# rcelha/rio-rs

Hardware: NVIDIA H100
Metric: placements/sec (higher is better)
Workload: dtype u32

## Files before the change

### rio_rs_b200/csrc/k_trie.cu

```cuda
#include "kernels.cuh"
#include "spec.cuh"
#include "bounded_tail.cuh"

#include <cstdlib>

namespace rio {

namespace {

constexpr int kTrieThreads = 256;
constexpr uint32_t kMaxLevels = 16;

__constant__ uint32_t c_lvl_s0[kMaxLevels];
__constant__ uint32_t c_lvl_m2[kMaxLevels];
__constant__ uint32_t c_lvl_h2[kMaxLevels];

__device__ __forceinline__ uint32_t smem_u32(const void *p) { return (uint32_t)__cvta_generic_to_shared(p); }

__device__ __forceinline__ void stage_blob_tma(void *smem_dst, const void *gsrc, uint32_t bytes, unsigned long long *bar) {
    if (threadIdx.x == 0) {
        asm volatile("mbarrier.init.shared::cta.b64 [%0], 1;" ::"r"(smem_u32(bar)) : "memory");
        asm volatile("fence.mbarrier_init.release.cluster;" ::: "memory");
    }
    __syncthreads();
    if (threadIdx.x == 0) {
        asm volatile("mbarrier.arrive.expect_tx.shared::cta.b64 _, [%0], %1;" ::"r"(smem_u32(bar)), "r"(bytes) : "memory");
        for (uint32_t off = 0; off < bytes; off += 32768u) {
            const uint32_t len = min(32768u, bytes - off);
            asm volatile("cp.async.bulk.shared::cluster.global.mbarrier::complete_tx::bytes [%0], [%1], %2, [%3];"
                         ::"r"(smem_u32(reinterpret_cast<unsigned char *>(smem_dst) + off)),
                           "l"(reinterpret_cast<const unsigned char *>(gsrc) + off), "r"(len), "r"(smem_u32(bar))
                         : "memory");
        }
    }
    uint32_t done = 0;
    while (!done) {
        asm volatile("{\n\t.reg .pred p;\n\tmbarrier.try_wait.parity.shared::cta.b64 p, [%1], %2;\n\tselp.u32 %0, 1, 0, p;\n\t}"
                     : "=r"(done) : "r"(smem_u32(bar)), "r"(0u) : "memory");
    }
}

__device__ __forceinline__ uint32_t walk_step(uint32_t off, uint32_t sel) {
    uint32_t r;
    asm("mad.lo.u32 %0, %1, 2, %2;" : "=r"(r) : "r"(off), "r"(sel));
    return r;
}

template <int BITS>
__device__ __forceinline__ uint32_t trie_leaf_index(ObjHash o, const uint32_t *__restrict__ tab32, uint32_t bits_rt) {
    uint32_t i = 1;
    if (BITS > 0) {
#pragma unroll
        for (int l = 0; l < BITS; l++) {
            const uint32_t u = contest_u(o, c_lvl_s0[l], c_lvl_m2[l], c_lvl_h2[l]);
            i = 2 * i + (u > tab32[i] ? 1u : 0u);
        }
    } else {
        for (uint32_t l = 0; l < bits_rt; l++) {
            const uint32_t u = contest_u(o, c_lvl_s0[l], c_lvl_m2[l], c_lvl_h2[l]);
            i = 2 * i + (u > tab32[i] ? 1u : 0u);
        }
    }
    return i;
}

__device__ __forceinline__ uint32_t trie_resolve_leaf(ObjHash o, uint32_t leaf, const unsigned char *__restrict__ blob) {
    if ((int32_t)leaf > -2) return leaf;
    uint32_t w = leaf;
    for (;;) {
        const unsigned char *p = blob + (w & 0x7FFFFFFFu);
        const uint4 r = *reinterpret_cast<const uint4 *>(p);
        const uint2 nn = *reinterpret_cast<const uint2 *>(p + 16);
        if (contest_u(o, r.x, r.y, r.z) <= r.w) return nn.x;
        if ((int32_t)nn.y >= 0) return nn.y;
        w = nn.y;
    }
}

struct TrieSmem {
    const uint32_t *tab32;
    const unsigned char *blob;
    uint32_t *hist;
};

template <bool SMEM>
__device__ __forceinline__ TrieSmem trie_stage(const TrieDev &t, uint32_t hist_bins) {
    extern __shared__ __align__(128) unsigned char smem_trie[];
    constexpr bool in_smem = SMEM;
    TrieSmem s;
    uint32_t off = 0;
    if (in_smem) {
        s.tab32 = reinterpret_cast<const uint32_t *>(smem_trie);
        s.blob = smem_trie;
        off = t.blob_bytes;
    } else {
        const unsigned char *g = reinterpret_cast<const unsigned char *>(t.blob);
        s.tab32 = reinterpret_cast<const uint32_t *>(g);
        s.blob = g;
    }
    s.hist = reinterpret_cast<uint32_t *>(smem_trie + off);
    for (uint32_t j = threadIdx.x; j < hist_bins; j += blockDim.x) s.hist[j] = 0;
    unsigned long long *bar = reinterpret_cast<unsigned long long *>(smem_trie + off + ((hist_bins * 4u + 15u) & ~15u));
    if (in_smem) stage_blob_tma(smem_trie, t.blob, t.blob_bytes, bar);
    else __syncthreads();
    return s;
}

template <int BITS, int OPT, int MODE, bool SMEM, int MINB = (SMEM ? 5 : 3)>
__global__ void __launch_bounds__(kTrieThreads, MINB)
k_assign_trie(const uint64_t *__restrict__ keys, uint64_t n, TrieDev t, uint32_t *__restrict__ out_idx, uint32_t *__restrict__ counters,
              uint32_t hist_bins, unsigned long long *__restrict__ moved, const __grid_constant__ BoundedTail tail) {
    static_assert(OPT % 2 == 0, "two objects per 128-bit load");
    constexpr bool in_smem = SMEM;
    constexpr int SEG = OPT / 2;
    const uint64_t tile_objs = (uint64_t)kTrieThreads * OPT;
    const uint64_t n_tiles = (n + tile_objs - 1) / tile_objs;
    unsigned long long n_moved = 0;
    ulonglong2 kk[SEG];
    auto load_tile = [&](uint64_t tile) {
        const uint64_t f0 = tile * tile_objs + 2 * threadIdx.x;
        if ((tile + 1) * tile_objs <= n) {
            const ulonglong2 *src = reinterpret_cast<const ulonglong2 *>(keys + f0);
#pragma unroll
            for (int g = 0; g < SEG; g++) kk[g] = __ldg(src + g * kTrieThreads);
            return;
        }
#pragma unroll
        for (int g = 0; g < SEG; g++) {
            const uint64_t f = f0 + (uint64_t)g * (2 * kTrieThreads);
            kk[g] = make_ulonglong2(0, 0);
            if (f + 1 < n) kk[g] = __ldg(reinterpret_cast<const ulonglong2 *>(keys + f));
            else if (f < n) kk[g].x = __ldg(keys + f);
        }
    };
    const TrieSmem s = trie_stage<SMEM>(t, hist_bins);
    asm volatile("griddepcontrol.launch_dependents;" ::: "memory");
    asm volatile("griddepcontrol.wait;" ::: "memory");
    if (blockIdx.x < n_tiles) load_tile(blockIdx.x);
    for (uint64_t tile = blockIdx.x; tile < n_tiles; tile += gridDim.x) {
        const uint64_t base = tile * tile_objs;
        const bool full_tile = base + tile_objs <= n;
        ObjHash o[OPT];
#pragma unroll
        for (int g = 0; g < SEG; g++) {
            o[2 * g] = obj_hash(kk[g].x);
            o[2 * g + 1] = obj_hash(kk[g].y);
        }
        if (tile + gridDim.x < n_tiles) load_tile(tile + gridDim.x);
        uint32_t leaf[OPT];
        if (in_smem) {
            const unsigned char *tb = reinterpret_cast<const unsigned char *>(s.tab32);
            uint32_t off[OPT];
#pragma unroll
            for (int k = 0; k < OPT; k++) off[k] = 4;
            if (BITS > 0) {
                constexpr int TOP = BITS >= 3 ? 3 : 0;
                if (TOP) {
#pragma unroll
                    for (int k = 0; k < OPT; k++) {
                        const bool c0 = contest_u(o[k], c_lvl_s0[0], c_lvl_m2[0], c_lvl_h2[0]) > t.top[1];
                        const bool c1 = contest_u(o[k], c_lvl_s0[1], c_lvl_m2[1], c_lvl_h2[1]) > (c0 ? t.top[3] : t.top[2]);
                        const uint32_t t2 = c0 ? (c1 ? t.top[7] : t.top[6]) : (c1 ? t.top[5] : t.top[4]);
                        const bool c2 = contest_u(o[k], c_lvl_s0[2], c_lvl_m2[2], c_lvl_h2[2]) > t2;
                        off[k] = 32u + (c0 ? 16u : 0u) + (c1 ? 8u : 0u) + (c2 ? 4u : 0u);
                    }
                }
#pragma unroll
                for (int l = TOP; l < BITS; l++) {
#pragma unroll
                    for (int k = 0; k < OPT; k++) {
                        const uint32_t u = contest_u(o[k], c_lvl_s0[l], c_lvl_m2[l], c_lvl_h2[l]);
                        const uint32_t thr = *reinterpret_cast<const uint32_t *>(tb + off[k]);
                        off[k] = walk_step(off[k], u > thr ? 4u : 0u);
                    }
                }
            } else {
                for (uint32_t l = 0; l < t.bits; l++) {
#pragma unroll
                    for (int k = 0; k < OPT; k++) {
                        const uint32_t u = contest_u(o[k], c_lvl_s0[l], c_lvl_m2[l], c_lvl_h2[l]);
                        const uint32_t thr = *reinterpret_cast<const uint32_t *>(tb + off[k]);
                        off[k] = walk_step(off[k], u > thr ? 4u : 0u);
                    }
                }
            }
#pragma unroll
            for (int k = 0; k < OPT; k++) leaf[k] = *reinterpret_cast<const uint32_t *>(tb + off[k]);
        } else {
#pragma unroll
            for (int k = 0; k < OPT; k++) leaf[k] = __ldg(s.tab32 + trie_leaf_index<0>(o[k], s.tab32, t.bits));
        }
        uint32_t nid[OPT];
#pragma unroll
        for (int k = 0; k < OPT; k++) nid[k] = trie_resolve_leaf(o[k], leaf[k], s.blob);
        if (MODE == 0 && full_tile) {
            uint2 *dst = reinterpret_cast<uint2 *>(out_idx + base + 2 * threadIdx.x);
#pragma unroll
            for (int g = 0; g < SEG; g++) dst[g * kTrieThreads] = make_uint2(nid[2 * g], nid[2 * g + 1]);
            if (counters && nid[0] != kNone) {
                if (hist_bins) {
#pragma unroll
                    for (int k = 0; k < OPT; k++) atomicAdd(&s.hist[nid[k]], 1u);
                } else {
#pragma unroll
                    for (int k = 0; k < OPT; k++) atomicAdd(&counters[nid[k]], 1u);
                }
            }
            continue;
        }
#pragma unroll
        for (int g = 0; g < SEG; g++) {
            const uint64_t first = base + (uint64_t)g * (2 * kTrieThreads) + 2 * threadIdx.x;
            if (first >= n) continue;
            const bool two = first + 1 < n;
            if (MODE == 1) {
                uint2 old = make_uint2(kNone, kNone);
                if (two) old = *reinterpret_cast<const uint2 *>(out_idx + first);
                else old.x = out_idx[first];
                const bool c0 = old.x != nid[2 * g], c1 = two && old.y != nid[2 * g + 1];
                if (c0 | c1) {
                    if (two) *reinterpret_cast<uint2 *>(out_idx + first) = make_uint2(nid[2 * g], nid[2 * g + 1]);
                    else out_idx[first] = nid[2 * g];
                }
                n_moved += (unsigned)c0 + (unsigned)c1;
            } else {
                if (two) *reinterpret_cast<uint2 *>(out_idx + first) = make_uint2(nid[2 * g], nid[2 * g + 1]);
                else out_idx[first] = nid[2 * g];
            }
            if (counters) {
                if (hist_bins) {
                    if (nid[2 * g] != kNone) atomicAdd(&s.hist[nid[2 * g]], 1u);
                    if (two && nid[2 * g + 1] != kNone) atomicAdd(&s.hist[nid[2 * g + 1]], 1u);
                } else {
                    if (nid[2 * g] != kNone) atomicAdd(&counters[nid[2 * g]], 1u);
                    if (two && nid[2 * g + 1] != kNone) atomicAdd(&counters[nid[2 * g + 1]], 1u);
                }
            }
        }
    }
    if (MODE == 1) {
#pragma unroll
        for (int sh = 16; sh > 0; sh >>= 1) n_moved += __shfl_xor_sync(0xFFFFFFFFu, n_moved, sh);
        if ((threadIdx.x & 31) == 0 && n_moved) atomicAdd(moved, n_moved);
    }
    if (hist_bins && counters) {
        __syncthreads();
        for (uint32_t j = threadIdx.x; j < hist_bins; j += blockDim.x) { const uint32_t v = s.hist[j]; if (v) atomicAdd(&counters[j], v); }
    }
    if (MODE == 0 && tail.enabled) {
        __shared__ uint32_t s_last;
        __threadfence();
        __syncthreads();
        if (threadIdx.x == 0) s_last = atomicAdd(tail.ticket, 1u) == gridDim.x - 1;
        __syncthreads();
        if (s_last) {
            if (threadIdx.x == 0) *tail.ticket = 0;
            __threadfence();
            exchange_and_check_block(tail, counters);
        }
    }
}

template <bool SMEM>
__global__ void __launch_bounds__(kTrieThreads, 4)
k_assign_trie_sel(const uint64_t *__restrict__ keys, const uint32_t *__restrict__ sel, uint64_t n_sel, TrieDev t, uint32_t *__restrict__ out_idx,
                  uint32_t *__restrict__ counters, uint32_t hist_bins) {
    const TrieSmem s = trie_stage<SMEM>(t, hist_bins);
    for (uint64_t q = (uint64_t)blockIdx.x * blockDim.x + threadIdx.x; q < n_sel; q += (uint64_t)gridDim.x * blockDim.x) {
        const uint32_t oi = __ldg(sel + q);
        const ObjHash o = obj_hash(__ldg(keys + oi));
        const uint32_t i = trie_leaf_index<0>(o, s.tab32, t.bits);
        const uint32_t nid = trie_resolve_leaf(o, s.tab32[i], s.blob);
        out_idx[oi] = nid;
        if (counters && nid != kNone) { if (hist_bins) atomicAdd(&s.hist[nid], 1u); else atomicAdd(&counters[nid], 1u); }
    }
    if (hist_bins && counters) {
        __syncthreads();
        for (uint32_t j = threadIdx.x; j < hist_bins; j += blockDim.x) { const uint32_t v = s.hist[j]; if (v) atomicAdd(&counters[j], v); }
    }
}

template <bool SMEM>
__global__ void __launch_bounds__(kTrieThreads, 4)
k_dir_reassign_trie(DirDev dir, TrieDev t, unsigned long long *__restrict__ moved) {
    const TrieSmem s = trie_stage<SMEM>(t, 0);
    const uint4 *slots = reinterpret_cast<const uint4 *>(dir.slots);
    const uint64_t cap = dir.mask + 1;
    unsigned long long n_moved = 0;
    for (uint64_t i = (uint64_t)blockIdx.x * blockDim.x + threadIdx.x; i < cap; i += (uint64_t)gridDim.x * blockDim.x) {
        const uint4 v = slots[i];
        const unsigned long long key = ((unsigned long long)v.y << 32) | v.x;
        if (key == kEmptyKey || v.z == kNone) continue;
        const ObjHash o = obj_hash(key);
        const uint32_t li = trie_leaf_index<0>(o, s.tab32, t.bits);
        const uint32_t nid = trie_resolve_leaf(o, s.tab32[li], s.blob);
        if (nid != v.z) { reinterpret_cast<uint32_t *>(&dir.slots[i].val)[0] = nid; n_moved++; }
    }
#pragma unroll
    for (int sh = 16; sh > 0; sh >>= 1) n_moved += __shfl_xor_sync(0xFFFFFFFFu, n_moved, sh);
    if ((threadIdx.x & 31) == 0 && n_moved) atomicAdd(moved, n_moved);
}

constexpr uint32_t kTrieSmemBudget = 200u * 1024u;

struct TrieLaunchShape { uint32_t hist_bins; uint32_t in_smem; size_t smem; int ctas_per_sm; };
TrieLaunchShape trie_shape(const TrieDev &t, bool want_hist, uint32_t n_total, int want_ctas) {
    TrieLaunchShape sh{};
    sh.hist_bins = (want_hist && n_total <= 8192) ? n_total : 0;
    const size_t tail = ((size_t)sh.hist_bins * 4 + 15) / 16 * 16 + 16;
    sh.in_smem = (t.blob_bytes + tail <= kTrieSmemBudget) ? 1u : 0u;
    sh.smem = (sh.in_smem ? t.blob_bytes : 0) + tail;
    int c = want_ctas;
    while (c > 1 && (size_t)c * (sh.smem + 1024) > 227u * 1024u) c--;
    sh.ctas_per_sm = c;
    return sh;
}

bool g_lvl_uploaded[64] = {};

}

void trie_upload_level_constants(int device) {
    if (device >= 0 && device < 64 && g_lvl_uploaded[device]) return;
    uint32_t s0[kMaxLevels], m2[kMaxLevels], h2[kMaxLevels];
    for (uint32_t l = 0; l < kMaxLevels; l++) {
        const ContestRec r = contest_rec(level_seed(l));
        s0[l] = r.s0; m2[l] = r.m2; h2[l] = r.h2;
    }
    cudaMemcpyToSymbol(c_lvl_s0, s0, sizeof s0);
    cudaMemcpyToSymbol(c_lvl_m2, m2, sizeof m2);
    cudaMemcpyToSymbol(c_lvl_h2, h2, sizeof h2);
    if (device >= 0 && device < 64) g_lvl_uploaded[device] = true;
}

uint64_t trie_wave_objects(int sm_count) { return (uint64_t)sm_count * 5 * kTrieThreads * 4; }

#define RIO_TRIE_LAUNCH(KERNEL, GRID, SMEM, ...)                                                                       \
    do {                                                                                                               \
        static bool attr_set[64] = {};    \
        int dev__ = 0;                                                                                                 \
        cudaGetDevice(&dev__);                                                                                         \
        if (dev__ < 0 || dev__ >= 64 || !attr_set[dev__]) {                                                            \
            cudaFuncSetAttribute(KERNEL, cudaFuncAttributeMaxDynamicSharedMemorySize, (int)kTrieSmemBudget + 1024);    \
            if (dev__ >= 0 && dev__ < 64) attr_set[dev__] = true;                                                      \
        }                                                                                                              \
        KERNEL<<<(GRID), kTrieThreads, (SMEM), L.stream>>>(__VA_ARGS__);                                               \
    } while (0)

#define RIO_TRIE_LAUNCH_PDL(KERNEL, GRID, SMEM, ...)                                                                   \
    do {                                                                                                               \
        static bool attr_set[64] = {};                                                                                 \
        static const bool pdl = [] { const char *e = getenv("RIO_TRIE_PDL"); return !(e && e[0] == '0'); }();          \
        int dev__ = 0;                                                                                                 \
        cudaGetDevice(&dev__);                                                                                         \
        if (dev__ < 0 || dev__ >= 64 || !attr_set[dev__]) {                                                            \
            cudaFuncSetAttribute(KERNEL, cudaFuncAttributeMaxDynamicSharedMemorySize, (int)kTrieSmemBudget + 1024);    \
            if (dev__ >= 0 && dev__ < 64) attr_set[dev__] = true;                                                      \
        }                                                                                                              \
        cudaLaunchConfig_t cfg__ = {};                                                                                 \
        cfg__.gridDim = dim3((unsigned)(GRID)); cfg__.blockDim = dim3(kTrieThreads);                                   \
        cfg__.dynamicSmemBytes = (SMEM); cfg__.stream = L.stream;                                                      \
        cudaLaunchAttribute at__[1];                                                                                   \
        at__[0].id = cudaLaunchAttributeProgrammaticStreamSerialization;                                               \
        at__[0].val.programmaticStreamSerializationAllowed = 1;                                                        \
        cfg__.attrs = at__; cfg__.numAttrs = pdl ? 1 : 0;                                                              \
        cudaLaunchKernelEx(&cfg__, KERNEL, __VA_ARGS__);                                                               \
    } while (0)

void launch_assign_trie(const Launch &L, const uint64_t *d_keys, uint64_t n, const TrieDev &t, uint32_t *d_out_idx, uint32_t *d_counters,
                        const uint32_t *d_sel, uint64_t n_sel, uint32_t n_total, const BoundedTail *tail) {
    BoundedTail no_tail{};
    const BoundedTail &tl = tail ? *tail : no_tail;
    const uint64_t n_work = d_sel ? n_sel : n;
    if (!n_work) return;
    if (d_sel) {
        const TrieLaunchShape sh = trie_shape(t, d_counters != nullptr, n_total, 4);
        const uint64_t blocks = (n_work + kTrieThreads - 1) / kTrieThreads, cap = (uint64_t)L.sm_count * sh.ctas_per_sm;
        const int grid = (int)(blocks < cap ? blocks : cap);
        if (sh.in_smem) RIO_TRIE_LAUNCH(k_assign_trie_sel<true>, grid, sh.smem, d_keys, d_sel, n_work, t, d_out_idx, d_counters, sh.hist_bins);
        else RIO_TRIE_LAUNCH(k_assign_trie_sel<false>, grid, sh.smem, d_keys, d_sel, n_work, t, d_out_idx, d_counters, sh.hist_bins);
    } else {
        constexpr int OPT = 4;
#ifdef RIO_ASSIGN_TUNING
        if (const char *tn = getenv("RIO_TRIE_TUNE")) {
            const int code = atoi(tn);
            auto go = [&](auto kern, int opt, int minb) {
                const TrieLaunchShape sh2 = trie_shape(t, d_counters != nullptr, n_total, minb);
                const uint64_t tiles2 = (n_work + (uint64_t)kTrieThreads * opt - 1) / ((uint64_t)kTrieThreads * opt), cap2 = (uint64_t)L.sm_count * sh2.ctas_per_sm;
                cudaFuncSetAttribute(kern, cudaFuncAttributeMaxDynamicSharedMemorySize, (int)kTrieSmemBudget + 1024);
                kern<<<(int)(tiles2 < cap2 ? tiles2 : cap2), kTrieThreads, sh2.smem, L.stream>>>(d_keys, n_work, t, d_out_idx, d_counters, sh2.hist_bins, nullptr, tl);
            };
            bool done = true;
            switch (code) {
                case 25: go(k_assign_trie<12, 2, 0, true, 5>, 2, 5); break;
                case 28: go(k_assign_trie<12, 2, 0, true, 8>, 2, 8); break;
                case 44: go(k_assign_trie<12, 4, 0, true, 4>, 4, 4); break;
                case 45: go(k_assign_trie<12, 4, 0, true, 5>, 4, 5); break;
                case 63: go(k_assign_trie<12, 6, 0, true, 3>, 6, 3); break;
                case 64: go(k_assign_trie<12, 6, 0, true, 4>, 6, 4); break;
                case 83: go(k_assign_trie<12, 8, 0, true, 3>, 8, 3); break;
                default: done = false;
            }
            if (done && t.bits == 12) { RIO_COUNT_LAUNCH(L); return; }
        }
#endif
        const TrieLaunchShape sh = trie_shape(t, d_counters != nullptr, n_total, 5);
        uint64_t cap = (uint64_t)L.sm_count * sh.ctas_per_sm;
        if (L.spare_ctas > 0 && cap > (uint64_t)L.spare_ctas + 1) cap -= (uint64_t)L.spare_ctas;
        const uint64_t tiles = (n_work + (uint64_t)kTrieThreads * OPT - 1) / ((uint64_t)kTrieThreads * OPT);
        const int grid = (int)(tiles < cap ? tiles : cap);
        unsigned long long *no_moved = nullptr;
        if (!sh.in_smem) RIO_TRIE_LAUNCH_PDL((k_assign_trie<0, OPT, 0, false>), grid, sh.smem, d_keys, n_work, t, d_out_idx, d_counters, sh.hist_bins, no_moved, tl);
        else if (t.bits == 12) RIO_TRIE_LAUNCH_PDL((k_assign_trie<12, OPT, 0, true>), grid, sh.smem, d_keys, n_work, t, d_out_idx, d_counters, sh.hist_bins, no_moved, tl);
        else RIO_TRIE_LAUNCH_PDL((k_assign_trie<0, OPT, 0, true>), grid, sh.smem, d_keys, n_work, t, d_out_idx, d_counters, sh.hist_bins, no_moved, tl);
    }
    RIO_COUNT_LAUNCH(L);
}

void launch_reassign_trie(const Launch &L, const uint64_t *d_keys, uint64_t n, const TrieDev &t, uint32_t *d_idx, uint32_t *d_counters,
                          uint32_t n_total, unsigned long long *d_moved) {
    if (!n) return;
    constexpr int OPT = 4;
 const TrieLaunchShape sh = trie_shape(t, d_counters != nullptr, n_total, 5);
    const uint64_t tiles = (n + (uint64_t)kTrieThreads * OPT - 1) / ((uint64_t)kTrieThreads * OPT), cap = (uint64_t)L.sm_count * sh.ctas_per_sm;
    const int grid = (int)(tiles < cap ? tiles : cap);
    if (!sh.in_smem) RIO_TRIE_LAUNCH((k_assign_trie<0, OPT, 1, false>), grid, sh.smem, d_keys, n, t, d_idx, d_counters, sh.hist_bins, d_moved, BoundedTail{});
    else if (t.bits == 12) RIO_TRIE_LAUNCH((k_assign_trie<12, OPT, 1, true>), grid, sh.smem, d_keys, n, t, d_idx, d_counters, sh.hist_bins, d_moved, BoundedTail{});
    else RIO_TRIE_LAUNCH((k_assign_trie<0, OPT, 1, true>), grid, sh.smem, d_keys, n, t, d_idx, d_counters, sh.hist_bins, d_moved, BoundedTail{});
    RIO_COUNT_LAUNCH(L);
}

void launch_dir_reassign_trie(const Launch &L, const DirDev &dir, const TrieDev &t, unsigned long long *d_moved) {
    const TrieLaunchShape sh = trie_shape(t, false, 0, 4);
    const uint64_t blocks = (dir.mask + 1 + kTrieThreads - 1) / kTrieThreads, cap = (uint64_t)L.sm_count * sh.ctas_per_sm;
    const int grid = (int)(blocks < cap ? blocks : cap);
    if (sh.in_smem) RIO_TRIE_LAUNCH(k_dir_reassign_trie<true>, grid, sh.smem, dir, t, d_moved);
    else RIO_TRIE_LAUNCH(k_dir_reassign_trie<false>, grid, sh.smem, dir, t, d_moved);
    RIO_COUNT_LAUNCH(L);
}

}
```

Measured before the change: 160.0 billion.

## Restructure trie assign kernel with register-cached top levels and interleaved walks

Rewrites the main trie assignment kernel. The top three heap levels are taken from registers (t.top) instead of shared memory. Each level step becomes a carry-based compare-and-double using a precomputed h2-1 constant table. The walks of all objects in a tile are interleaved level by level for ILP, and the ragged last tile is split into a noinline tail function so the hot loop has no bounds checks. The previous kernel is kept behind a tuning macro. The risks are the new TrieDev.top field dependency, more register pressure, and counting hist for the whole tile only when nid[0] != kNone, which looks like it changes counter semantics.

```diff
diff --git a/rio_rs_b200/csrc/k_trie.cu b/rio_rs_b200/csrc/k_trie.cu
--- a/rio_rs_b200/csrc/k_trie.cu
+++ b/rio_rs_b200/csrc/k_trie.cu
@@ -2,6 +2,7 @@
 #include "spec.cuh"
 #include "bounded_tail.cuh"
 
+#include <cassert>
 #include <cstdlib>
 
 namespace rio {
@@ -14,6 +15,7 @@
 __constant__ uint32_t c_lvl_s0[kMaxLevels];
 __constant__ uint32_t c_lvl_m2[kMaxLevels];
 __constant__ uint32_t c_lvl_h2[kMaxLevels];
+__constant__ uint32_t c_lvl_h2e[kMaxLevels];
 
 __device__ __forceinline__ uint32_t smem_u32(const void *p) { return (uint32_t)__cvta_generic_to_shared(p); }
 
@@ -38,12 +40,6 @@
         asm volatile("{\n\t.reg .pred p;\n\tmbarrier.try_wait.parity.shared::cta.b64 p, [%1], %2;\n\tselp.u32 %0, 1, 0, p;\n\t}"
                      : "=r"(done) : "r"(smem_u32(bar)), "r"(0u) : "memory");
     }
-}
-
-__device__ __forceinline__ uint32_t walk_step(uint32_t off, uint32_t sel) {
-    uint32_t r;
-    asm("mad.lo.u32 %0, %1, 2, %2;" : "=r"(r) : "r"(off), "r"(sel));
-    return r;
 }
 
 template <int BITS>
@@ -84,21 +80,22 @@
 };
 
 template <bool SMEM>
+__device__ __forceinline__ TrieSmem trie_view(const void *gblob, uint32_t blob_bytes) {
+    extern __shared__ __align__(128) unsigned char smem_trie[];
+    const unsigned char *b = SMEM ? smem_trie : reinterpret_cast<const unsigned char *>(gblob);
+    TrieSmem s;
+    s.tab32 = reinterpret_cast<const uint32_t *>(b);
+    s.blob = b;
+    s.hist = reinterpret_cast<uint32_t *>(smem_trie + (SMEM ? blob_bytes : 0u));
+    return s;
+}
+
+template <bool SMEM>
 __device__ __forceinline__ TrieSmem trie_stage(const TrieDev &t, uint32_t hist_bins) {
     extern __shared__ __align__(128) unsigned char smem_trie[];
     constexpr bool in_smem = SMEM;
-    TrieSmem s;
-    uint32_t off = 0;
-    if (in_smem) {
-        s.tab32 = reinterpret_cast<const uint32_t *>(smem_trie);
-        s.blob = smem_trie;
-        off = t.blob_bytes;
-    } else {
-        const unsigned char *g = reinterpret_cast<const unsigned char *>(t.blob);
-        s.tab32 = reinterpret_cast<const uint32_t *>(g);
-        s.blob = g;
-    }
-    s.hist = reinterpret_cast<uint32_t *>(smem_trie + off);
+    const TrieSmem s = trie_view<SMEM>(t.blob, t.blob_bytes);
+    const uint32_t off = in_smem ? t.blob_bytes : 0u;
     for (uint32_t j = threadIdx.x; j < hist_bins; j += blockDim.x) s.hist[j] = 0;
     unsigned long long *bar = reinterpret_cast<unsigned long long *>(smem_trie + off + ((hist_bins * 4u + 15u) & ~15u));
     if (in_smem) stage_blob_tma(smem_trie, t.blob, t.blob_bytes, bar);
@@ -106,9 +103,196 @@
     return s;
 }
 
+__device__ __forceinline__ uint32_t heap_step(uint32_t i, uint32_t ue, uint32_t t3) {
+    uint32_t r;
+    asm("{\n\t.reg .u32 c;\n\tsub.cc.u32 c, %1, %2;\n\taddc.u32 %0, %3, %3;\n\t}" : "=r"(r) : "r"(ue), "r"(t3), "r"(i));
+    return r;
+}
+
+struct TrieTop { uint32_t t1, t2, t3, t4, t5, t6, t7; };
+
+template <int BITS, int OPT, bool SMEM>
+__device__ __forceinline__ void trie_walk_tile(const ObjHash (&o)[OPT], const TrieSmem &s, const TrieTop &top, uint32_t bits_rt, uint32_t (&leaf)[OPT]) {
+    if (!SMEM) {
+#pragma unroll
+        for (int k = 0; k < OPT; k++) leaf[k] = __ldg(s.tab32 + trie_leaf_index<0>(o[k], s.tab32, bits_rt));
+        return;
+    }
+    uint32_t i[OPT];
+    constexpr int TOP = BITS >= 3 ? 3 : 0;
+#pragma unroll
+    for (int k = 0; k < OPT; k++) {
+        if (TOP) {
+            const bool c0 = contest_u(o[k], c_lvl_s0[0], c_lvl_m2[0], c_lvl_h2[0]) > top.t1;
+            const bool c1 = contest_u(o[k], c_lvl_s0[1], c_lvl_m2[1], c_lvl_h2[1]) > (c0 ? top.t3 : top.t2);
+            const uint32_t t2 = c0 ? (c1 ? top.t7 : top.t6) : (c1 ? top.t5 : top.t4);
+            i[k] = heap_step(4u + (c0 ? 2u : 0u) + (c1 ? 1u : 0u), contest_u(o[k], c_lvl_s0[2], c_lvl_m2[2], c_lvl_h2e[2]), t2);
+        } else {
+            i[k] = 1;
+        }
+    }
+    if (BITS > 0) {
+#pragma unroll
+        for (int l = TOP; l < BITS; l++) {
+#pragma unroll
+            for (int k = 0; k < OPT; k++) i[k] = heap_step(i[k], contest_u(o[k], c_lvl_s0[l], c_lvl_m2[l], c_lvl_h2e[l]), s.tab32[i[k]]);
+        }
+    } else {
+        for (uint32_t l = 0; l < bits_rt; l++) {
+#pragma unroll
+            for (int k = 0; k < OPT; k++) i[k] = heap_step(i[k], contest_u(o[k], c_lvl_s0[l], c_lvl_m2[l], c_lvl_h2e[l]), s.tab32[i[k]]);
+        }
+    }
+#pragma unroll
+    for (int k = 0; k < OPT; k++) leaf[k] = s.tab32[i[k]];
+}
+
+template <int BITS, int OPT, int MODE, bool SMEM>
+__device__ __noinline__ unsigned long long trie_tail_tile(const uint64_t *__restrict__ keys, uint64_t n, uint64_t base, const void *gblob,
+                                                          uint32_t blob_bytes, uint32_t bits, uint32_t *__restrict__ out_idx,
+                                                          uint32_t *__restrict__ counters, uint32_t hist_bins) {
+    constexpr int SEG = OPT / 2;
+    const TrieSmem s = trie_view<SMEM>(gblob, blob_bytes);
+    const uint32_t *h = s.tab32;
+    const TrieTop top{h[1], h[2], h[3], h[4], h[5], h[6], h[7]};
+    ObjHash o[OPT];
+#pragma unroll
+    for (int g = 0; g < SEG; g++) {
+        const uint64_t f = base + (uint64_t)g * (2 * kTrieThreads) + 2 * threadIdx.x;
+        ulonglong2 kk = make_ulonglong2(0, 0);
+        if (f + 1 < n) kk = __ldg(reinterpret_cast<const ulonglong2 *>(keys + f));
+        else if (f < n) kk.x = __ldg(keys + f);
+        o[2 * g] = obj_hash(kk.x);
+        o[2 * g + 1] = obj_hash(kk.y);
+    }
+    uint32_t nid[OPT];
+    trie_walk_tile<BITS, OPT, SMEM>(o, s, top, bits, nid);
+#pragma unroll
+    for (int k = 0; k < OPT; k++) nid[k] = trie_resolve_leaf(o[k], nid[k], s.blob);
+    unsigned long long n_moved = 0;
+#pragma unroll
+    for (int g = 0; g < SEG; g++) {
+        const uint64_t first = base + (uint64_t)g * (2 * kTrieThreads) + 2 * threadIdx.x;
+        if (first >= n) continue;
+        const bool two = first + 1 < n;
+        if (MODE == 1) {
+            uint2 old = make_uint2(kNone, kNone);
+            if (two) old = *reinterpret_cast<const uint2 *>(out_idx + first);
+            else old.x = out_idx[first];
+            const bool c0 = old.x != nid[2 * g], c1 = two && old.y != nid[2 * g + 1];
+            if (c0 | c1) {
+                if (two) *reinterpret_cast<uint2 *>(out_idx + first) = make_uint2(nid[2 * g], nid[2 * g + 1]);
+                else out_idx[first] = nid[2 * g];
+            }
+            n_moved += (unsigned)c0 + (unsigned)c1;
+        } else {
+            if (two) *reinterpret_cast<uint2 *>(out_idx + first) = make_uint2(nid[2 * g], nid[2 * g + 1]);
+            else out_idx[first] = nid[2 * g];
+        }
+        if (counters) {
+            if (hist_bins) {
+                if (nid[2 * g] != kNone) atomicAdd(&s.hist[nid[2 * g]], 1u);
+                if (two && nid[2 * g + 1] != kNone) atomicAdd(&s.hist[nid[2 * g + 1]], 1u);
+            } else {
+                if (nid[2 * g] != kNone) atomicAdd(&counters[nid[2 * g]], 1u);
+                if (two && nid[2 * g + 1] != kNone) atomicAdd(&counters[nid[2 * g + 1]], 1u);
+            }
+        }
+    }
+    return n_moved;
+}
+
 template <int BITS, int OPT, int MODE, bool SMEM, int MINB = (SMEM ? 5 : 3)>
 __global__ void __launch_bounds__(kTrieThreads, MINB)
 k_assign_trie(const uint64_t *__restrict__ keys, uint64_t n, TrieDev t, uint32_t *__restrict__ out_idx, uint32_t *__restrict__ counters,
+              uint32_t hist_bins, unsigned long long *__restrict__ moved, const __grid_constant__ BoundedTail tail) {
+    static_assert(OPT % 2 == 0, "two objects per 128-bit load");
+    constexpr int SEG = OPT / 2;
+    constexpr uint32_t tile_objs = (uint32_t)kTrieThreads * OPT;
+    const uint32_t n_full = (uint32_t)(n / tile_objs);
+    const TrieTop top{t.top[1], t.top[2], t.top[3], t.top[4], t.top[5], t.top[6], t.top[7]};
+    unsigned long long n_moved = 0;
+    ulonglong2 kk[SEG];
+    auto load_tile = [&](uint32_t tile) {
+        const ulonglong2 *src = reinterpret_cast<const ulonglong2 *>(keys + (size_t)tile * tile_objs + 2 * threadIdx.x);
+#pragma unroll
+        for (int g = 0; g < SEG; g++) kk[g] = __ldg(src + g * kTrieThreads);
+    };
+    const TrieSmem s = trie_stage<SMEM>(t, hist_bins);
+    asm volatile("griddepcontrol.launch_dependents;" ::: "memory");
+    asm volatile("griddepcontrol.wait;" ::: "memory");
+    uint32_t tile = blockIdx.x;
+    if (tile < n_full) load_tile(tile);
+    for (; tile < n_full; tile += gridDim.x) {
+        ObjHash o[OPT];
+#pragma unroll
+        for (int g = 0; g < SEG; g++) {
+            o[2 * g] = obj_hash(kk[g].x);
+            o[2 * g + 1] = obj_hash(kk[g].y);
+        }
+        if (tile + gridDim.x < n_full) load_tile(tile + gridDim.x);
+        uint32_t nid[OPT];
+        trie_walk_tile<BITS, OPT, SMEM>(o, s, top, t.bits, nid);
+#pragma unroll
+        for (int k = 0; k < OPT; k++) nid[k] = trie_resolve_leaf(o[k], nid[k], s.blob);
+        uint2 *dst = reinterpret_cast<uint2 *>(out_idx + (size_t)tile * tile_objs + 2 * threadIdx.x);
+#pragma unroll
+        for (int g = 0; g < SEG; g++) {
+            const uint2 v = make_uint2(nid[2 * g], nid[2 * g + 1]);
+            if (MODE == 1) {
+                const uint2 old = dst[g * kTrieThreads];
+                const bool c0 = old.x != v.x, c1 = old.y != v.y;
+                if (c0 | c1) dst[g * kTrieThreads] = v;
+                n_moved += (unsigned)c0 + (unsigned)c1;
+            } else {
+                dst[g * kTrieThreads] = v;
+            }
+        }
+        if (counters && nid[0] != kNone) {
+            if (hist_bins) {
+#pragma unroll
+                for (int k = 0; k < OPT; k++) atomicAdd(&s.hist[nid[k]], 1u);
+            } else {
+#pragma unroll
+                for (int k = 0; k < OPT; k++) atomicAdd(&counters[nid[k]], 1u);
+            }
+        }
+    }
+    if (tile == n_full && (uint64_t)n_full * tile_objs < n)
+        n_moved += trie_tail_tile<BITS, OPT, MODE, SMEM>(keys, n, (uint64_t)n_full * tile_objs, t.blob, t.blob_bytes, t.bits, out_idx, counters, hist_bins);
+    if (MODE == 1) {
+#pragma unroll
+        for (int sh = 16; sh > 0; sh >>= 1) n_moved += __shfl_xor_sync(0xFFFFFFFFu, n_moved, sh);
+        if ((threadIdx.x & 31) == 0 && n_moved) atomicAdd(moved, n_moved);
+    }
+    if (hist_bins && counters) {
+        __syncthreads();
+        for (uint32_t j = threadIdx.x; j < hist_bins; j += blockDim.x) { const uint32_t v = s.hist[j]; if (v) atomicAdd(&counters[j], v); }
+    }
+    if (MODE == 0 && tail.enabled) {
+        __shared__ uint32_t s_last;
+        __threadfence();
+        __syncthreads();
+        if (threadIdx.x == 0) s_last = atomicAdd(tail.ticket, 1u) == gridDim.x - 1;
+        __syncthreads();
+        if (s_last) {
+            if (threadIdx.x == 0) *tail.ticket = 0;
+            __threadfence();
+            exchange_and_check_block(tail, counters);
+        }
+    }
+}
+
+#ifdef RIO_ASSIGN_TUNING
+__device__ __forceinline__ uint32_t walk_step(uint32_t off, uint32_t sel) {
+    uint32_t r;
+    asm("mad.lo.u32 %0, %1, 2, %2;" : "=r"(r) : "r"(off), "r"(sel));
+    return r;
+}
+
+template <int BITS, int OPT, int MODE, bool SMEM, int MINB = (SMEM ? 5 : 3)>
+__global__ void __launch_bounds__(kTrieThreads, MINB)
+k_assign_trie_prev(const uint64_t *__restrict__ keys, uint64_t n, TrieDev t, uint32_t *__restrict__ out_idx, uint32_t *__restrict__ counters,
               uint32_t hist_bins, unsigned long long *__restrict__ moved, const __grid_constant__ BoundedTail tail) {
     static_assert(OPT % 2 == 0, "two objects per 128-bit load");
     constexpr bool in_smem = SMEM;
@@ -260,6 +444,7 @@
         }
     }
 }
+#endif
 
 template <bool SMEM>
 __global__ void __launch_bounds__(kTrieThreads, 4)
@@ -316,20 +501,27 @@
     return sh;
 }
 
+uint64_t trie_tiles(uint64_t n, int opt) {
+    const uint64_t tile = (uint64_t)kTrieThreads * opt, tiles = (n + tile - 1) / tile;
+    assert(tiles < (1ull << 31));
+    return tiles;
+}
+
 bool g_lvl_uploaded[64] = {};
 
 }
 
 void trie_upload_level_constants(int device) {
     if (device >= 0 && device < 64 && g_lvl_uploaded[device]) return;
-    uint32_t s0[kMaxLevels], m2[kMaxLevels], h2[kMaxLevels];
+    uint32_t s0[kMaxLevels], m2[kMaxLevels], h2[kMaxLevels], h2e[kMaxLevels];
     for (uint32_t l = 0; l < kMaxLevels; l++) {
         const ContestRec r = contest_rec(level_seed(l));
-        s0[l] = r.s0; m2[l] = r.m2; h2[l] = r.h2;
+        s0[l] = r.s0; m2[l] = r.m2; h2[l] = r.h2; h2e[l] = r.h2 - 1u;
     }
     cudaMemcpyToSymbol(c_lvl_s0, s0, sizeof s0);
     cudaMemcpyToSymbol(c_lvl_m2, m2, sizeof m2);
     cudaMemcpyToSymbol(c_lvl_h2, h2, sizeof h2);
+    cudaMemcpyToSymbol(c_lvl_h2e, h2e, sizeof h2e);
     if (device >= 0 && device < 64) g_lvl_uploaded[device] = true;
 }
 
@@ -386,7 +578,7 @@
             const int code = atoi(tn);
             auto go = [&](auto kern, int opt, int minb) {
                 const TrieLaunchShape sh2 = trie_shape(t, d_counters != nullptr, n_total, minb);
-                const uint64_t tiles2 = (n_work + (uint64_t)kTrieThreads * opt - 1) / ((uint64_t)kTrieThreads * opt), cap2 = (uint64_t)L.sm_count * sh2.ctas_per_sm;
+                const uint64_t tiles2 = trie_tiles(n_work, opt), cap2 = (uint64_t)L.sm_count * sh2.ctas_per_sm;
                 cudaFuncSetAttribute(kern, cudaFuncAttributeMaxDynamicSharedMemorySize, (int)kTrieSmemBudget + 1024);
                 kern<<<(int)(tiles2 < cap2 ? tiles2 : cap2), kTrieThreads, sh2.smem, L.stream>>>(d_keys, n_work, t, d_out_idx, d_counters, sh2.hist_bins, nullptr, tl);
             };
@@ -407,9 +599,16 @@
         const TrieLaunchShape sh = trie_shape(t, d_counters != nullptr, n_total, 5);
         uint64_t cap = (uint64_t)L.sm_count * sh.ctas_per_sm;
         if (L.spare_ctas > 0 && cap > (uint64_t)L.spare_ctas + 1) cap -= (uint64_t)L.spare_ctas;
-        const uint64_t tiles = (n_work + (uint64_t)kTrieThreads * OPT - 1) / ((uint64_t)kTrieThreads * OPT);
+        const uint64_t tiles = trie_tiles(n_work, OPT);
         const int grid = (int)(tiles < cap ? tiles : cap);
         unsigned long long *no_moved = nullptr;
+#ifdef RIO_ASSIGN_TUNING
+        if (const char *tn = getenv("RIO_TRIE_TUNE"); tn && atoi(tn) == 1 && sh.in_smem && t.bits == 12) {
+            RIO_TRIE_LAUNCH_PDL((k_assign_trie_prev<12, OPT, 0, true>), grid, sh.smem, d_keys, n_work, t, d_out_idx, d_counters, sh.hist_bins, no_moved, tl);
+            RIO_COUNT_LAUNCH(L);
+            return;
+        }
+#endif
         if (!sh.in_smem) RIO_TRIE_LAUNCH_PDL((k_assign_trie<0, OPT, 0, false>), grid, sh.smem, d_keys, n_work, t, d_out_idx, d_counters, sh.hist_bins, no_moved, tl);
         else if (t.bits == 12) RIO_TRIE_LAUNCH_PDL((k_assign_trie<12, OPT, 0, true>), grid, sh.smem, d_keys, n_work, t, d_out_idx, d_counters, sh.hist_bins, no_moved, tl);
         else RIO_TRIE_LAUNCH_PDL((k_assign_trie<0, OPT, 0, true>), grid, sh.smem, d_keys, n_work, t, d_out_idx, d_counters, sh.hist_bins, no_moved, tl);
@@ -421,8 +620,8 @@
                           uint32_t n_total, unsigned long long *d_moved) {
     if (!n) return;
     constexpr int OPT = 4;
- const TrieLaunchShape sh = trie_shape(t, d_counters != nullptr, n_total, 5);
-    const uint64_t tiles = (n + (uint64_t)kTrieThreads * OPT - 1) / ((uint64_t)kTrieThreads * OPT), cap = (uint64_t)L.sm_count * sh.ctas_per_sm;
+    const TrieLaunchShape sh = trie_shape(t, d_counters != nullptr, n_total, 5);
+    const uint64_t tiles = trie_tiles(n, OPT), cap = (uint64_t)L.sm_count * sh.ctas_per_sm;
     const int grid = (int)(tiles < cap ? tiles : cap);
     if (!sh.in_smem) RIO_TRIE_LAUNCH((k_assign_trie<0, OPT, 1, false>), grid, sh.smem, d_keys, n, t, d_idx, d_counters, sh.hist_bins, d_moved, BoundedTail{});
     else if (t.bits == 12) RIO_TRIE_LAUNCH((k_assign_trie<12, OPT, 1, true>), grid, sh.smem, d_keys, n, t, d_idx, d_counters, sh.hist_bins, d_moved, BoundedTail{});
```

Result: no change. 162.3 billion, median of 6 (+1.4%).
